# mj129/Tramba

Measured on AMD Instinct MI355X. Metric: images/sec fwd Tramba-V 384x384, higher is better.
Workload: dtype bf16; 1 GPU; Tramba-V (VMamba-B encoder) 384x384 bf16 inference, batch 4 per GPU, random-init weights (seed 1026), randn images; global_batch=4, launch=hipGraph replay, decoder guide branches on a side stream

## Files before the change

include/tramba_hip.h:

```cpp
#ifndef TRAMBA_HIP_H
#define TRAMBA_HIP_H

#include <stddef.h>
#include <stdint.h>

#ifdef __cplusplus
extern "C" {
#endif

typedef enum { TRAMBA_F32 = 0, TRAMBA_F16 = 1, TRAMBA_BF16 = 2 } tramba_dtype;

typedef enum {
    TRAMBA_SCAN_RASTER = 0,
    TRAMBA_SCAN_LINE = 1,
    TRAMBA_SCAN_HELIX = 2,
    TRAMBA_SCAN_WINDOW = 3,
    TRAMBA_SCAN_DILATION = 4
} tramba_scan_family;

typedef enum { TRAMBA_ACT_NONE = 0, TRAMBA_ACT_SILU = 1, TRAMBA_ACT_GELU = 2,
               TRAMBA_ACT_SIGMOID_GATE = 3 ,
               TRAMBA_ACT_GELU_GRAD_MUL = 4
             } tramba_act;

#define TRAMBA_OK 0
#define TRAMBA_ERR_ARG (-1)
#define TRAMBA_ERR_UNSUPPORTED (-2)
#define TRAMBA_ERR_HIP (-3)

const char *tramba_last_error(void);
int tramba_abi_version(void);
int tramba_device_error(void);
int tramba_profile_enable(int which, int enable);
int tramba_profile_read(int which, double *total_ms, double *total_bytes);
int tramba_profile_min_units(int which, double min_units);
int tramba_tune_set(int knob, int value);
int tramba_tune_get(int knob);
#define TRAMBA_TUNE_MERGE_FORM 0
#define TRAMBA_TUNE_SCAN_FORM 1
#define TRAMBA_TUNE_SCAN_W 2
#define TRAMBA_TUNE_GEMM_TILE 3
#define TRAMBA_TUNE_MAILBOX_SKIP 4
#define TRAMBA_TUNE_DW_FORM 6
#define TRAMBA_TUNE_DW_ROWS 7
#define TRAMBA_TUNE_COUNT 8
#define TRAMBA_PROF_SCAN_BOUNDARY 0
#define TRAMBA_PROF_SCAN_FUSED 1
#define TRAMBA_PROF_GEMM 2
#define TRAMBA_PROF_MERGE 3
#define TRAMBA_PROF_SCAN_BWD 4
#define TRAMBA_PROF_WGRAD 5
#define TRAMBA_PROF_LAYERNORM 6
#define TRAMBA_PROF_DW 7
#define TRAMBA_PROF_COUNT 8

int tramba_scan_family_k(int family);
int tramba_default_window(int h);
int tramba_scan_table(int family, int h, int w, int param, int32_t *out);
int tramba_scan_table_inverse(const int32_t *table, int k, int l, int32_t *inv_ptr, int32_t *inv_idx);

int tramba_selective_scan_nchunk(int l, int io_dtype);
int tramba_selective_scan_fwd(const void *u, const void *delta, const float *A, const void *Bm,
                              const void *Cm, const float *D, const float *delta_bias, void *out,
                              float *ckpt, int batch, int kd, int k, int n, int l, int io_dtype,
                              int out_dtype, int delta_softplus, void *stream);
int tramba_selective_scan_bwd(const void *u, const void *delta, const float *A, const void *Bm,
                              const void *Cm, const float *D, const float *delta_bias,
                              const float *dout, const float *ckpt, void *du, void *ddelta,
                              float *dA, float *dB, float *dC, float *dD, float *ddelta_bias,
                              int batch, int kd, int k, int n, int l, int io_dtype,
                              int delta_softplus, int ncopy, void *stream);

int tramba_cross_scan(const void *x, const int32_t *table, void *xs, int batch, int c, int l, int k,
                      int dtype, void *stream);
int tramba_cross_merge(const void *ys, const int32_t *inv_ptr, const int32_t *inv_idx, void *y,
                       int batch, int c, int l, int k, int dtype, void *stream);

int tramba_ss2d_group_stride(int r);
size_t tramba_ss2d_scan_workspace(int batch, int l, int d, int k);
int tramba_ss2d_scan_cl(const void *x, const float *xdbl, const int32_t *table, const float *dt_w,
                        const float *dt_bias, const float *A, const float *Ds, void *ys, void *workspace,
                        size_t workspace_bytes, int batch, int l, int d, int k, int r, int dtype,
                        int ys_dtype, float *states, int a_log, void *stream);
size_t tramba_ss2d_scan_bwd_workspace(int batch, int l, int d, int k);
int tramba_ss2d_scan_bwd_cl(const void *x, const float *xdbl, const int32_t *table, const float *dt_w,
                            const float *dt_bias, const float *A, const float *Ds, const void *gym, void *gu,
                            void *graw, float *gB, float *gC, int bc_stride, float *gpar, void *workspace,
                            size_t workspace_bytes, int have_states, int batch, int l, int d, int k, int r, int dtype,
                            int gym_dtype, int flags, void *stream);
#define TRAMBA_SCAN_BWD_A_LOG 1
#define TRAMBA_SCAN_BWD_BC_PARTIALS 2
int tramba_ss2d_bwd_prep_cl(const float *xdbl, const int32_t *table, const float *bpart, const float *cpart, void *ranks,
                            float *gseq, int batch, int l, int k, int r, int ctiles, int dtype, void *stream);
int tramba_ss2d_bwd_assemble_cl(const float *gseq, const int32_t *inv_ptr, const int32_t *inv_idx, void *out, int batch,
                                int l, int k, int r, int dtype, void *stream);
int tramba_ss2d_merge_norm_cl(const void *ys, const int32_t *inv_ptr, const int32_t *inv_idx,
                              const float *ln_w, const float *ln_b, void *y, int batch, int l, int d,
                              int k, float eps, int act, int ys_dtype, int dtype, void *stream);
// ... 152 lines not shown
```

tramba_amd/csrc/linear.hip:

```cpp
#include <stdlib.h>
#include <string.h>

#include <type_traits>

#include "common.h"

namespace tramba {

typedef __attribute__((ext_vector_type(8))) short frag8_t;
typedef __attribute__((ext_vector_type(8))) _Float16 frag8h_t;
typedef __attribute__((ext_vector_type(16))) float acc16_t;

template <typename T> struct Mfma;
template <> struct Mfma<__hip_bfloat16> {
    static constexpr int KSTEP = 16;
    using frag = frag8_t;
    static __device__ __forceinline__ acc16_t run(frag a, frag b, acc16_t c)
    {
        typedef __attribute__((ext_vector_type(8))) __bf16 bf8;
        return __builtin_amdgcn_mfma_f32_32x32x16_bf16(__builtin_bit_cast(bf8, a), __builtin_bit_cast(bf8, b), c, 0, 0, 0);
    }
};
template <> struct Mfma<__half> {
    static constexpr int KSTEP = 16;
// ... 715 lines not shown
        acc[0][0] = Mfma<T>::run(b[2], a[2], acc[0][0]);
        asm volatile("s_waitcnt lgkmcnt(0)" : "+v"(a[3]), "+v"(b[3]) : : "memory");
        acc[0][0] = Mfma<T>::run(b[3], a[3], acc[0][0]);
    };
    int kt0 = 0;
    for (; kt0 + NSTG <= nk; kt0 += NSTG) {
        kstep(kt0, std::integral_constant<int, 0>{});
        kstep(kt0 + 1, std::integral_constant<int, 1>{});
        if constexpr (NSTG > 2) kstep(kt0 + 2, std::integral_constant<int, 2>{});
        if constexpr (NSTG > 3) kstep(kt0 + 3, std::integral_constant<int, 3>{});
        if constexpr (NSTG > 4) {
            kstep(kt0 + 4, std::integral_constant<int, 4>{});
            kstep(kt0 + 5, std::integral_constant<int, 5>{});
            kstep(kt0 + 6, std::integral_constant<int, 6>{});
            kstep(kt0 + 7, std::integral_constant<int, 7>{});
        }
    }
    if (kt0 < nk) kstep(kt0, std::integral_constant<int, 0>{});
    if constexpr (NSTG > 2) {
        if (kt0 + 1 < nk) kstep(kt0 + 1, std::integral_constant<int, 1>{});
    }
    if constexpr (NSTG > 3) {
        if (kt0 + 2 < nk) kstep(kt0 + 2, std::integral_constant<int, 2>{});
    }
    if constexpr (NSTG > 4) {
        if (kt0 + 3 < nk) kstep(kt0 + 3, std::integral_constant<int, 3>{});
        if (kt0 + 4 < nk) kstep(kt0 + 4, std::integral_constant<int, 4>{});
        if (kt0 + 5 < nk) kstep(kt0 + 5, std::integral_constant<int, 5>{});
        if (kt0 + 6 < nk) kstep(kt0 + 6, std::integral_constant<int, 6>{});
    }
    __syncthreads();
    if constexpr (LNIN) {
        float2 *rowstat = reinterpret_cast<float2 *>(lds + LDS_BYTES);
#pragma unroll
        for (int i = 0; i < 2; ++i) {
            float s1 = rs1[i], s2 = rs2[i];
#pragma unroll
            for (int m = 1; m < 8; m <<= 1) {
                s1 += __shfl_xor(s1, m, 64);
                s2 += __shfl_xor(s2, m, 64);
            }
            const float mean = s1 / (float)K;
            const float var = fmaxf(s2 / (float)K - mean * mean, 0.f);
            if ((tid & 7) == 0) rowstat[(tid >> 3) + 32 * i] = make_float2(mean, rsqrtf(var + li.eps));
        }
        tile_epilogue<T, TO, BM, BN>(acc, lds, bias, res, y, M, N, act, m0, n0, li.colsum,
                                     reinterpret_cast<const float2 *>(lds + LDS_BYTES));
    } else {
        tile_epilogue<T, TO, BM, BN>(acc, lds, bias, res, y, M, N, act, m0, n0, nullptr, nullptr, DUAL ? y_pre : nullptr);
    }
#endif
}

#define TRAMBA_DSR128_(OUT, ADDR, OFF) asm volatile("ds_read_b128 %0, %1 offset:" #OFF : "=v"(OUT) : "v"(ADDR) : "memory")
template <typename T, typename TO, int NSTG, bool LNIN = false, bool DUAL = false>
__global__ __launch_bounds__(512) void linear_pc_kernel(const T *__restrict__ x, const T *__restrict__ w,
                                                       const float *__restrict__ bias, const T *__restrict__ res,
                                                       TO *__restrict__ y, long M, int N, int K, int act,
                                                       LnIn li = LnIn{nullptr, 0.f}, TO *__restrict__ y_pre = nullptr)
{
#if defined(__HIP_DEVICE_COMPILE__)
    constexpr int BM = 64, BN = 64;
    constexpr int TILE_BYTES = (BM + BN) * kBK * 2;
    constexpr int EPI_BYTES = BM * (BN + 4) * 4;
    constexpr int LDS_BYTES = NSTG * TILE_BYTES > EPI_BYTES ? NSTG * TILE_BYTES : EPI_BYTES;
    static_assert(NSTG == 3 || NSTG == 4, "stage index = kt % NSTG with the loop unrolled by NSTG");
    __shared__ __attribute__((aligned(1024))) unsigned char lds[LDS_BYTES + (LNIN ? BM * 8 : 0)];
    typedef __attribute__((address_space(3))) void lds_void;

    const int tid = threadIdx.x, lane = tid & 63;
    const int wave = __builtin_amdgcn_readfirstlane(tid >> 6);
    const bool loader = wave >= 4;
    const int cw = wave & 3;
    const int wm = cw >> 1, wn = cw & 1;
    const int r32 = lane & 31, hi = lane >> 5;
    long m0;
    int n0;
    {
        const unsigned nblk = gridDim.x * gridDim.y, lin = blockIdx.y * gridDim.x + blockIdx.x;
        const unsigned q = nblk >> 3, r = nblk & 7, xcd = lin & 7, slot = lin >> 3;
        const unsigned t = xcd * q + (xcd < r ? xcd : r) + slot;
        m0 = (long)(t / gridDim.x) * BM;
        n0 = (int)(t % gridDim.x) * BN;
    }
    const int nk = K / kBK;
    const unsigned rowb = (unsigned)K * 2u;
    const long mrows = M - m0 < BM ? M - m0 : BM;
    const int nrows = N - n0 < BN ? N - n0 : BN;
    const bool stage_b = cw >= 2;
    const __amdgpu_buffer_rsrc_t rs = stage_b ? make_rsrc(w + (long)n0 * K, (unsigned)nrows * rowb)
                                              : make_rsrc(x + m0 * K, (unsigned)mrows * rowb);
    unsigned voff[4];
#pragma unroll
    for (int j = 0; j < 4; ++j) {
        const int row = ((cw & 1) * 4 + j) * 8 + (lane >> 3);
        const int c = (lane & 7) ^ ((row >> 1) & 7);
        voff[j] = (unsigned)row * rowb + (unsigned)c * 16u;
    }
    unsigned char *mine = lds + (stage_b ? BM * kBK * 2 : 0) + (cw & 1) * 4096;
    auto issue = [&](int kt, int stg) {
        const unsigned so = (unsigned)kt * (kBK * 2);
#pragma unroll
        for (int j = 0; j < 4; ++j)
            __builtin_amdgcn_raw_ptr_buffer_load_lds(rs, (lds_void *)(mine + stg * TILE_BYTES + j * 1024), 16, voff[j], so, 0,
                                                     0);
    };
    const unsigned lbase = (unsigned)(size_t)(__attribute__((address_space(3))) unsigned char *)lds;
    unsigned aad[4], bad[4];
    {
        const int ra_ = wm * 32 + r32, rb_ = wn * 32 + r32;
        const unsigned a0 = lbase + (unsigned)(ra_ * 128 + ((hi ^ ((ra_ >> 1) & 7)) * 16));
        const unsigned b0 = lbase + (unsigned)(BM * kBK * 2 + rb_ * 128 + ((hi ^ ((rb_ >> 1) & 7)) * 16));
#pragma unroll
        for (int kk = 0; kk < 4; ++kk) {
            aad[kk] = a0 ^ (unsigned)(kk * 32);
            bad[kk] = b0 ^ (unsigned)(kk * 32);
        }
    }
    acc16_t acc[1][1];
#pragma unroll
    for (int r = 0; r < 16; ++r) acc[0][0][r] = 0.f;
    const int lt = tid & 255;
    float rs1[2] = {0.f, 0.f}, rs2[2] = {0.f, 0.f};
    const unsigned sad = lbase + (unsigned)((lt >> 3) * 128 + (lt & 7) * 16);

    constexpr int DEPTH = NSTG - 1;
    if (loader) {
#pragma unroll
        for (int t = 0; t < DEPTH; ++t)
            if (t < nk) issue(t, t);
    }
    auto kstep = [&](int kt, auto stg_c) {
        constexpr int STG = decltype(stg_c)::value;
        if (loader) {
            const int later = nk - 1 - kt;
            if (later >= DEPTH - 1) {
                if constexpr (DEPTH == 2) asm volatile("s_waitcnt vmcnt(4)" ::: "memory");
                else asm volatile("s_waitcnt vmcnt(8)" ::: "memory");
            } else {
                switch (later) {
                case 0: asm volatile("s_waitcnt vmcnt(0)" ::: "memory"); break;
                default: asm volatile("s_waitcnt vmcnt(4)" ::: "memory"); break;
                }
            }
        }
        __builtin_amdgcn_s_barrier();
        asm volatile("" ::: "memory");
        if (loader) {
            if (kt + DEPTH < nk) issue(kt + DEPTH, (STG + DEPTH) % NSTG);
        } else {
            frag8_t a[4], b[4];
            v4u_t sv[2];
            if constexpr (LNIN) {
                if constexpr (STG == 0) { TRAMBA_DSR128_(sv[0], sad, 0); TRAMBA_DSR128_(sv[1], sad, 4096); }
                else if constexpr (STG == 1) { TRAMBA_DSR128_(sv[0], sad, 16384); TRAMBA_DSR128_(sv[1], sad, 20480); }
                else if constexpr (STG == 2) { TRAMBA_DSR128_(sv[0], sad, 32768); TRAMBA_DSR128_(sv[1], sad, 36864); }
                else { TRAMBA_DSR128_(sv[0], sad, 49152); TRAMBA_DSR128_(sv[1], sad, 53248); }
            }
#define TRAMBA_RD_STG_(S)                                                                            \
    TRAMBA_DSR128_(a[0], aad[0], S); TRAMBA_DSR128_(b[0], bad[0], S); TRAMBA_DSR128_(a[1], aad[1], S); \
    TRAMBA_DSR128_(b[1], bad[1], S); TRAMBA_DSR128_(a[2], aad[2], S); TRAMBA_DSR128_(b[2], bad[2], S); \
    TRAMBA_DSR128_(a[3], aad[3], S); TRAMBA_DSR128_(b[3], bad[3], S)
// ... 366 lines not shown
    return ncw;
}

template <typename T, int K, bool LNIN, bool DUAL, bool RES>
static void launch_ws(int ncw, const void *x, const void *w, const float *bias, const void *res, void *y, long m, int n, int act,
                      LnIn li, void *y_pre, hipStream_t s)
{
    const int npanel = n / (128 * ncw);
    const long t32 = (m + 31) / 32;
    const long resident = 256L * (K == 128 ? 3 : 2);
    long gt = resident / npanel;
    if (gt > t32) gt = t32;
    if (gt < 1) gt = 1;
    dim3 grid((unsigned)(gt * npanel)), block(256);
#define WS_(NCW_)                                                                                                      \
    hipLaunchKernelGGL((linear_ws_kernel<T, K, NCW_, LNIN, DUAL, RES>), grid, block, 0, s, (const T *)x, (const T *)w, bias, \
                       (const T *)res, (T *)y, m, n, act, li, (T *)y_pre, npanel, (int)gt)
    if constexpr (K == 128) {
        if (ncw == 2) { WS_(2); } else { WS_(1); }
    } else {
        WS_(1);
    }
#undef WS_
}

template <typename T, bool LNIN, bool DUAL>
static void launch_ws_k(int ncw, const void *x, const void *w, const float *bias, const void *res, void *y, long m, int n, int k,
                        int act, LnIn li, void *y_pre, hipStream_t s)
{
    if (k == 128) {
        if (res) { if constexpr (!DUAL) launch_ws<T, 128, LNIN, false, true>(ncw, x, w, bias, res, y, m, n, act, li, y_pre, s); }
        else launch_ws<T, 128, LNIN, DUAL, false>(ncw, x, w, bias, res, y, m, n, act, li, y_pre, s);
    } else {
        if (res) { if constexpr (!DUAL) launch_ws<T, 256, LNIN, false, true>(ncw, x, w, bias, res, y, m, n, act, li, y_pre, s); }
        else launch_ws<T, 256, LNIN, DUAL, false>(ncw, x, w, bias, res, y, m, n, act, li, y_pre, s);
    }
}

constexpr int DMA_SHORT_K = 256;

enum GemmKind { GEMM_PLAIN = 0, GEMM_LN = 1, GEMM_DUAL = 2, GEMM_TWO_SRC, GEMM_CONV };
enum class GemmForm {
    WS,
    PC3, PC4,
    DMA2, DMA3, DMA4,
    LEAN,
    TILED128, TILED64, TILED64_PF3
};
struct GemmPlan {
    GemmForm form;
    int ncw;
};

static GemmPlan gemm_plan(GemmKind kind, long m, int n, int k, int act, bool same_dtype)
{
    if (kind == GEMM_TWO_SRC) return {GemmForm::LEAN, 0};
    if (kind == GEMM_CONV || k % 64 != 0 || (double)k * 2.0 * 128.0 >= 2147483648.0) {
        const long big = ((m + 127) / 128) * ((n + 127) / 128);
        if (big >= 2048 && k >= 1024) return {GemmForm::TILED128, 0};
        return {k <= 128 ? GemmForm::TILED64 : GemmForm::TILED64_PF3, 0};
    }
    int tune = tramba_tune_get(TRAMBA_TUNE_GEMM_TILE);
    if (tune == 7 && kind != GEMM_PLAIN) tune = 0;
    if (tune == 0 || tune == 19) {
        const bool ws_act = act == TRAMBA_ACT_NONE || act == TRAMBA_ACT_GELU || act == TRAMBA_ACT_SILU;
        const int ncw = same_dtype && ws_act ? ws_ncw(m, n, k) : 0;
        if (ncw && (tune == 19 ? m >= 64 : ws_rule(m, n, k, kind))) return {GemmForm::WS, ncw};
    }
    switch (tune) {
    case 7: return {GemmForm::DMA4, 0};
    case 13: return {GemmForm::DMA2, 0};
    case 14: return {GemmForm::DMA3, 0};
    case 16: return {GemmForm::PC3, 0};
    case 17: return {GemmForm::PC4, 0};
    }
    const long tiles64 = ((m + 63) / 64) * ((n + 63) / 64);
    const int pc = tune == 18 ? 0 : pc_rule(tiles64, k, kind);
    if (pc) return {pc == 4 ? GemmForm::PC4 : GemmForm::PC3, 0};
    if (k <= DMA_SHORT_K && tiles64 >= 1024) return {GemmForm::DMA2, 0};
    if (kind == GEMM_PLAIN && tiles64 <= 256 && k >= 1024) return {GemmForm::DMA4, 0};
    return {GemmForm::DMA3, 0};
}

struct GemmArgs {
    const void *x, *w;
    const float *bias;
    const void *res;
    void *y;
    long m;
    int n, k, act;
    LnIn li{nullptr, 0.f};
    void *y_pre = nullptr;
    const void *x2 = nullptr;
    int k1 = 0;
    ConvGeom cg{0, 0, 0, 0, 0};
};

template <typename T, typename TO, bool LNIN = false, bool DUAL = false, bool CONV = false>
static void launch_gemm(const GemmPlan &p, const GemmArgs &a, hipStream_t s)
{
    const T *x = (const T *)a.x, *w = (const T *)a.w, *res = (const T *)a.res;
    TO *y = (TO *)a.y, *y_pre = (TO *)a.y_pre;
    const long m = a.m;
    const int n = a.n, k = a.k, act = a.act;
    const dim3 g64((n + 63) / 64, (unsigned)((m + 63) / 64)), g128((n + 127) / 128, (unsigned)((m + 127) / 128));
    switch (p.form) {
    case GemmForm::WS:
        launch_ws_k<T, LNIN, DUAL>(p.ncw, a.x, a.w, a.bias, a.res, a.y, m, n, k, act, a.li, a.y_pre, s);
        break;
    case GemmForm::PC3:
        hipLaunchKernelGGL((linear_pc_kernel<T, TO, 3, LNIN, DUAL>), g64, dim3(512), 0, s, x, w, a.bias, res, y, m, n, k, act, a.li, y_pre);
        break;
    case GemmForm::PC4:
        hipLaunchKernelGGL((linear_pc_kernel<T, TO, 4, LNIN, DUAL>), g64, dim3(512), 0, s, x, w, a.bias, res, y, m, n, k, act, a.li, y_pre);
        break;
    case GemmForm::DMA2:
        hipLaunchKernelGGL((linear_dma_kernel<T, TO, 2, LNIN, DUAL>), g64, dim3(256), 0, s, x, w, a.bias, res, y, m, n, k, act, a.li, y_pre);
        break;
    case GemmForm::DMA3:
        hipLaunchKernelGGL((linear_dma_kernel<T, TO, 3, LNIN, DUAL>), g64, dim3(256), 0, s, x, w, a.bias, res, y, m, n, k, act, a.li, y_pre);
        break;
    case GemmForm::DMA4:
        if constexpr (!LNIN && !DUAL)
            hipLaunchKernelGGL((linear_dma_kernel<T, TO, 4>), g64, dim3(256), 0, s, x, w, a.bias, res, y, m, n, k, act, a.li, y_pre);
        break;
    case GemmForm::LEAN:
        hipLaunchKernelGGL((linear_lean_kernel<T, TO, 64, 64, 1>), g64, dim3(256), 0, s, x, w, a.bias, res, y, m, n, k, act,
                           (const T *)a.x2, a.k1);
        break;
    case GemmForm::TILED128:
        hipLaunchKernelGGL((linear_tiled_kernel<T, TO, 128, 128, 2, CONV>), g128, dim3(256), 0, s, x, w, a.bias, res, y, m, n, k, act, a.cg);
        break;
    case GemmForm::TILED64:
        hipLaunchKernelGGL((linear_tiled_kernel<T, TO, 64, 64, 1, CONV>), g64, dim3(256), 0, s, x, w, a.bias, res, y, m, n, k, act, a.cg);
        break;
    case GemmForm::TILED64_PF3:
        hipLaunchKernelGGL((linear_tiled_kernel<T, TO, 64, 64, 3, CONV>), g64, dim3(256), 0, s, x, w, a.bias, res, y, m, n, k, act, a.cg);
        break;
    }
}

template <bool LNIN = false>
static void launch_gemm16(const GemmPlan &p, const GemmArgs &a, int dtype, int out_dtype, hipStream_t s)
{
    if (dtype == TRAMBA_BF16) {
        if (out_dtype == TRAMBA_F32) launch_gemm<__hip_bfloat16, float, LNIN>(p, a, s);
        else launch_gemm<__hip_bfloat16, __hip_bfloat16, LNIN>(p, a, s);
    } else {
        if (out_dtype == TRAMBA_F32) launch_gemm<__half, float, LNIN>(p, a, s);
        else launch_gemm<__half, __half, LNIN>(p, a, s);
    }
}

template <typename TO>
__global__ __launch_bounds__(256) void linear32_kernel(const float *__restrict__ x, const float *__restrict__ w,
                                                      const float *__restrict__ bias, const float *__restrict__ res,
                                                      TO *__restrict__ y, long M, int N, int K, int act)
{
    const int lane = threadIdx.x & 63, wave = threadIdx.x >> 6;
    const long m0 = (long)blockIdx.y * 128 + (wave >> 1) * 64;
    const int n0 = blockIdx.x * 128 + (wave & 1) * 64;
    if (m0 >= M || n0 >= N) return;
    acc16_t acc[2][2];
#pragma unroll
    for (int i = 0; i < 2; ++i)
#pragma unroll
        for (int j = 0; j < 2; ++j)
#pragma unroll
// ... 114 lines not shown
                 "linear2_cl: tensors must be 16-byte aligned");
    TRAMBA_CHECK((m + 63) / 64 <= 65535 && (double)k * 2.0 * 128.0 < 2147483648.0, "linear2_cl: shape exceeds this build's limits");
    hipStream_t s = (hipStream_t)stream;
    ProfScope prof(TRAMBA_PROF_GEMM, s, 2.0 * (double)m * n * k);
    GemmArgs a{x1, w, bias, residual, y, m, n, k, act};
    a.x2 = x2;
    a.k1 = k1;
    launch_gemm16(gemm_plan(GEMM_TWO_SRC, m, n, k, act, out_dtype == dtype), a, dtype, out_dtype, s);
    TRAMBA_LAUNCH_CHECK();
    return TRAMBA_OK;
}

extern "C" int tramba_expand_norm_head_cl(const void *x, const void *w, const float *ln_w, const float *ln_b,
                                          const float *head_w, float head_b, float *y, int batch, int h, int wd, int cin,
                                          int p, float eps, int dtype, void *stream)
{
    TRAMBA_CHECK(x && w && ln_w && ln_b && head_w && y, "expand_norm_head_cl: null tensor");
    TRAMBA_CHECK(batch > 0 && h > 0 && wd > 0 && cin > 0 && p > 0, "expand_norm_head_cl: empty shape");
    TRAMBA_CHECK(dtype == TRAMBA_BF16 || dtype == TRAMBA_F16, "expand_norm_head_cl: 16-bit dtypes only");
    TRAMBA_CHECK(cin % 64 == 0, "expand_norm_head_cl: Cin=%d must be a multiple of 64", cin);
    TRAMBA_CHECK(aligned16(x) && aligned16(w), "expand_norm_head_cl: tensors must be 16-byte aligned");
    const long m = (long)batch * h * wd;
    const int n = p * p * 128;
    TRAMBA_CHECK(m < 2147483647L && (m + 63) / 64 <= 65535, "expand_norm_head_cl: too many pixels");
    hipStream_t s = (hipStream_t)stream;
    ProfScope prof(TRAMBA_PROF_GEMM, s, 2.0 * (double)m * n * cin);
    const LnHead hd{ln_w, ln_b, head_w, head_b, eps, h, wd, p, y};
    dim3 grid((unsigned)(n / 128), (unsigned)((m + 63) / 64)), block(256);
    if (dtype == TRAMBA_BF16) {
        using T = __hip_bfloat16;
        hipLaunchKernelGGL((linear_lean_kernel<T, T, 64, 128, 1, true>), grid, block, 0, s, (const T *)x, (const T *)w,
                           (const float *)nullptr, (const T *)nullptr, (T *)nullptr, m, n, cin, 0, (const T *)nullptr, 0, hd);
    } else {
        using T = __half;
        hipLaunchKernelGGL((linear_lean_kernel<T, T, 64, 128, 1, true>), grid, block, 0, s, (const T *)x, (const T *)w,
                           (const float *)nullptr, (const T *)nullptr, (T *)nullptr, m, n, cin, 0, (const T *)nullptr, 0, hd);
    }
    TRAMBA_LAUNCH_CHECK();
    return TRAMBA_OK;
}

extern "C" int tramba_conv3x3s2_cl(const void *x, const void *w, const float *bias, void *y, int batch, int hin,
                                   int win, int cin, int cout, int dtype, void *stream)
{
    TRAMBA_CHECK(x && w && y, "conv3x3s2_cl: null tensor");
    TRAMBA_CHECK(batch > 0 && hin > 0 && win > 0 && cin > 0 && cout > 0, "conv3x3s2_cl: empty shape");
    TRAMBA_CHECK(cin % 64 == 0, "conv3x3s2_cl: Cin=%d must be a multiple of 64", cin);
    TRAMBA_CHECK(dtype == TRAMBA_BF16 || dtype == TRAMBA_F16, "conv3x3s2_cl: bf16/f16 only (fp32 convs run on MIOpen)");
    TRAMBA_CHECK(aligned16(x) && aligned16(w) && aligned16(y), "conv3x3s2_cl: tensors must be 16-byte aligned");
    ConvGeom cg{hin, win, cin, (hin + 1) / 2, (win + 1) / 2};
    const long m = (long)batch * cg.hout * cg.wout;
    TRAMBA_CHECK((m + 63) / 64 <= 65535, "conv3x3s2_cl: too many output pixels");
    hipStream_t s = (hipStream_t)stream;
    const GemmPlan p = gemm_plan(GEMM_CONV, m, cout, 9 * cin, TRAMBA_ACT_NONE, true);
    GemmArgs a{x, w, bias, nullptr, y, m, cout, 9 * cin, TRAMBA_ACT_NONE};
    a.cg = cg;
    if (dtype == TRAMBA_BF16) launch_gemm<__hip_bfloat16, __hip_bfloat16, false, false, true>(p, a, s);
    else launch_gemm<__half, __half, false, false, true>(p, a, s);
    TRAMBA_LAUNCH_CHECK();
    return TRAMBA_OK;
}

extern "C" int tramba_linear_dual_cl(const void *x, const void *w, const float *bias, void *y_pre, void *y_act, int64_t m,
                                     int n, int k, int act, int dtype, void *stream)
{
    TRAMBA_CHECK(x && w && y_pre && y_act, "linear_dual_cl: null tensor");
    TRAMBA_CHECK(m > 0 && n > 0 && k > 0, "linear_dual_cl: empty shape");
    TRAMBA_CHECK(dtype == TRAMBA_BF16 || dtype == TRAMBA_F16, "linear_dual_cl: 16-bit activations only");
    TRAMBA_CHECK(act == TRAMBA_ACT_GELU || act == TRAMBA_ACT_SILU, "linear_dual_cl: act must be GELU or SiLU");
    TRAMBA_CHECK(k % 64 == 0 && n % 8 == 0 && (double)k * 2.0 * 128.0 < 2147483648.0 && (m + 63) / 64 <= 65535,
                 "linear_dual_cl: needs K %% 64 == 0, N %% 8 == 0");
    TRAMBA_CHECK(aligned16(x) && aligned16(w) && aligned16(y_pre) && aligned16(y_act), "linear_dual_cl: 16-byte alignment");
    hipStream_t s = (hipStream_t)stream;
    ProfScope prof(TRAMBA_PROF_GEMM, s, 2.0 * (double)m * n * k);
    const GemmPlan p = gemm_plan(GEMM_DUAL, m, n, k, act, true);
    GemmArgs a{x, w, bias, nullptr, y_act, m, n, k, act};
    a.y_pre = y_pre;
    if (dtype == TRAMBA_BF16) launch_gemm<__hip_bfloat16, __hip_bfloat16, false, true>(p, a, s);
    else launch_gemm<__half, __half, false, true>(p, a, s);
    TRAMBA_LAUNCH_CHECK();
    return TRAMBA_OK;
}
```

tramba_amd/csrc/ss2d_fused.hip:

```cpp
#include <stdlib.h>
#include <string.h>

#include <type_traits>

#include "common.h"
#include "norm.h"

namespace tramba {

constexpr int kMaxW = 8;

typedef __attribute__((ext_vector_type(8))) short frag8_t;
typedef __attribute__((ext_vector_type(8))) __bf16 bf16x8_t;
typedef __attribute__((ext_vector_type(16))) float acc16_t;

constexpr int kTP = 32;

__host__ __device__ inline int xdbl_rank_pad(int r) { return (r + 7) & ~7; }
__host__ __device__ inline int xdbl_group_stride(int r) { return xdbl_rank_pad(r) + 4; }
inline double rg_bytes(int r) { return 4.0 * xdbl_group_stride(r); }

template <bool SPLIT>
__device__ __forceinline__ void pack_frag(const float (&v)[8], frag8_t &hi, frag8_t &lo)
{
// ... 1628 lines not shown
    case 1: BWD_(T, 1, SP_); break;    \
    case 2: BWD_(T, 2, SP_); break;    \
    case 3: BWD_(T, 3, SP_); break;    \
    default: BWD_(T, 4, SP_); break;   \
    }
    if (dtype == TRAMBA_F32) { BWD_NK_(float, true) }
    else if (dtype == TRAMBA_BF16) { BWD_NK_(__hip_bfloat16, false) }
    else if (dtype == TRAMBA_F16) { BWD_NK_(__half, false) }
    else {
        set_error("ss2d_scan_bwd_cl: bad dtype %d", dtype);
        return TRAMBA_ERR_ARG;
    }
#undef BWD_NK_
#undef BWD_
#undef BWD_G_
    TRAMBA_LAUNCH_CHECK();
    return TRAMBA_OK;
}

extern "C" int tramba_ss2d_merge_norm_cl(const void *ys, const int32_t *inv_ptr, const int32_t *inv_idx,
                                         const float *ln_w, const float *ln_b, void *y, int batch, int l,
                                         int d, int k, float eps, int act, int ys_dtype, int dtype,
                                         void *stream)
{
    return tramba_ss2d_merge_grad_cl(ys, inv_ptr, inv_idx, ln_w, ln_b, y, nullptr, nullptr, batch, l, d, k, eps, act, ys_dtype,
                                     dtype, stream);
}

extern "C" int tramba_ss2d_merge_grad_cl(const void *ys, const int32_t *inv_ptr, const int32_t *inv_idx,
                                         const float *ln_w, const float *ln_b, void *y, const void *addend,
                                         const void *zpre, int batch, int l, int d, int k, float eps, int act,
                                         int ys_dtype, int dtype, void *stream)
{
    TRAMBA_CHECK(ys && inv_ptr && inv_idx && y && (eps < 0.f || (ln_w && ln_b)), "ss2d_merge_norm_cl: null tensor");
    TRAMBA_CHECK((!addend && !zpre) || (eps < 0.f && zpre && aligned16(zpre) && (!addend || aligned16(addend))),
                 "ss2d_merge_grad_cl: the SiLU-gradient epilogue belongs to a merge-only call (eps < 0) and needs zpre");
    TRAMBA_CHECK(batch > 0 && l > 0 && d > 0 && k > 0, "ss2d_merge_norm_cl: empty shape");
    TRAMBA_CHECK(ys_dtype == TRAMBA_F32 || ys_dtype == dtype, "ss2d_merge_norm_cl: ys must be f32 or dtype");
    hipStream_t s = (hipStream_t)stream;
    const long npix = (long)batch * l;
    TRAMBA_CHECK(npix < 2147483647L, "ss2d_merge_norm_cl: B*L exceeds the 32-bit pixel index of this build");
    int v = (d % 4 == 0) ? 4 : ((d % 2 == 0) ? 2 : 1);
    TRAMBA_CHECK((d + kWave * v - 1) / (kWave * v) <= kNormMaxIt, "ss2d_merge_norm_cl: D=%d too large", d);
    TRAMBA_CHECK(aligned16(ys) && aligned16(y), "ss2d_merge_norm_cl: tensors must be 16-byte aligned");
    const int nit_need = (d + kWave * v - 1) / (kWave * v);
    const int nit = nit_need <= 1 ? 1 : (nit_need <= 2 ? 2 : (nit_need <= 4 ? 4 : 8));
    ProfScope prof(TRAMBA_PROF_MERGE, s, (double)batch * k * l * (double)d * dtype_size(ys_dtype) +
                                              (double)batch * l * (double)d * dtype_size(dtype));
    const bool sum_only = eps < 0.f;
    const int tune = tramba_tune_get(TRAMBA_TUNE_MERGE_FORM);
    const bool stream_ok = !sum_only && nit <= 2 && k <= 8 && (double)k * l * d * 4.0 < 4294967296.0;
    const bool stream_form = stream_ok && (tune == 2 || (tune == 0 && k <= 4 && npix >= 8192));
    const bool wide = k > 4;
    const int pw = wide ? 4 : 16;
    const int nchunk = (l + pw - 1) / pw;
    const long nwaves = (long)batch * nchunk;
    int hs = 0;
    if (wide) {
        hs = 1;
        while ((long)hs * hs < l) ++hs;
        if ((long)hs * hs != l || hs % pw != 0) hs = 0;
    }
    const bool split_form = !sum_only && !stream_form && tune != 1 && (ys_dtype == TRAMBA_F32 || k <= 4) && nit >= 4 &&
                            npix <= 16384;
    if (!stream_form && !split_form) {
        const int vd = norm_vec(d, ys_dtype == TRAMBA_F32 ? 4 : 8);
        const int nd_need = (d + kWave * vd - 1) / (kWave * vd);
        TRAMBA_CHECK(nd_need <= kNormMaxIt, "ss2d_merge_norm_cl: D=%d too large", d);
        TRAMBA_CHECK((double)k * l * d * 4.0 < 4294967296.0, "ss2d_merge_norm_cl: K*L*D too large for 32-bit offsets");
        const int nd = nd_need <= 1 ? 1 : (nd_need <= 2 ? 2 : (nd_need <= 4 ? 4 : 8));
        int hh = 1;
        while ((long)hh * hh < l) ++hh;
        if ((long)hh * hh != l) hh = 0;
        dim3 gridd((unsigned)((npix + 3) / 4)), blockd(256);
#define DEEP_(TY, T, V_, N_)                                                                                      \
    hipLaunchKernelGGL((ss2d_merge_norm_deep_kernel<TY, T, V_, N_>), gridd, blockd, 0, s, (const TY *)ys, inv_ptr, \
                       inv_idx, ln_w, ln_b, (T *)y, npix, batch, l, d, k, hh, eps, act, (const T *)addend, (const T *)zpre)
#define DEEP_N_(TY, T, V_)                    \
    if (nd == 1) { DEEP_(TY, T, V_, 1); }     \
    else if (nd == 2) { DEEP_(TY, T, V_, 2); } \
    else if (nd == 4) { DEEP_(TY, T, V_, 4); } \
    else { DEEP_(TY, T, V_, 8); }
#define DEEP_V_(TY, T)                                                  \
    if (vd == 8) {                                                      \
        if constexpr (sizeof(TY) == 2) { DEEP_N_(TY, T, 8) }            \
    } else if (vd == 4) { DEEP_N_(TY, T, 4) }                           \
    else if (vd == 2) { DEEP_N_(TY, T, 2) }                             \
    else { DEEP_N_(TY, T, 1) }
        TRAMBA_DISPATCH_DTYPE(dtype, T, {
            if (ys_dtype == TRAMBA_F32) { DEEP_V_(float, T) } else { DEEP_V_(T, T) }
        });
#undef DEEP_V_
#undef DEEP_N_
#undef DEEP_
        TRAMBA_LAUNCH_CHECK();
        return TRAMBA_OK;
    }
    dim3 grid(stream_form ? (unsigned)((nwaves + 3) / 4) : (unsigned)npix), block(256);
#define GO_(TY, T, V_, N_)                                                                                    \
    if (split_form)                                                                                           \
        hipLaunchKernelGGL((ss2d_merge_norm_split_kernel<TY, T, V_, (N_ >= 4 ? N_ : 4), 4>), grid, block, 0, s, \
                           (const TY *)ys, inv_ptr, inv_idx, ln_w, ln_b, (T *)y, npix, l, d, k, eps, act);    \
    else if (wide)                                                                                            \
        hipLaunchKernelGGL((ss2d_merge_norm_stream_kernel<TY, T, V_, (N_ <= 2 ? N_ : 2), 8>), grid, block, 0, s, \
                           (const TY *)ys, inv_ptr, inv_idx, ln_w, ln_b, (T *)y, nwaves, nchunk, pw, l, d, k, eps, \
                           act, batch, hs);                                                                   \
    else                                                                                                      \
// ... 24 lines not shown
```

tramba_amd/hip.py:

```python
import ctypes
import os
import threading
import weakref

import numpy as np
import torch

_HERE = os.path.dirname(os.path.abspath(__file__))
LIB_PATH = os.path.join(_HERE, "_lib", "libtramba_hip.so")

F32, F16, BF16 = 0, 1, 2
ACT_NONE, ACT_SILU, ACT_GELU, ACT_SIGMOID_GATE, ACT_GELU_GRAD_MUL = 0, 1, 2, 3, 4
SCAN_RASTER, SCAN_LINE, SCAN_HELIX, SCAN_WINDOW, SCAN_DILATION = range(5)
FAMILY = {"raster": SCAN_RASTER, "line": SCAN_LINE, "helix": SCAN_HELIX, "window": SCAN_WINDOW,
          "dilation": SCAN_DILATION}
PROF_SCAN_BOUNDARY, PROF_SCAN_FUSED, PROF_GEMM, PROF_MERGE, PROF_SCAN_BWD, PROF_WGRAD, PROF_LAYERNORM, PROF_DW = 0, 1, 2, 3, 4, 5, 6, 7

_DT = {torch.float32: F32, torch.float16: F16, torch.bfloat16: BF16}

c_int, c_i64, c_f, c_vp = ctypes.c_int, ctypes.c_int64, ctypes.c_float, ctypes.c_void_p

SIGNATURES = {
    "tramba_last_error": (ctypes.c_char_p, []),
    "tramba_abi_version": (c_int, []),
# ... 172 lines not shown
        return conv
    _f32_cache[key] = (ver, conv, ref)
    return conv


_table_cache = {}


def default_window(h: int) -> int:
    return lib().tramba_default_window(h)


def scan_table_host(family: str, h: int, w: int = None, param: int = 0) -> np.ndarray:
    w = h if w is None else w
    fam = FAMILY[family]
    k = _check(lib().tramba_scan_family_k(fam), "scan_family_k")
    out = np.empty((k, h * w), dtype=np.int32)
    _check(lib().tramba_scan_table(fam, h, w, param, out.ctypes.data), f"scan_table({family},{h})")
    return out


def scan_table_inverse_host(table: np.ndarray):
    k, l = table.shape
    table = np.ascontiguousarray(table, dtype=np.int32)
    ptr = np.empty(l + 1, dtype=np.int32)
    idx = np.empty(k * l, dtype=np.int32)
    _check(lib().tramba_scan_table_inverse(table.ctypes.data, k, l, ptr.ctypes.data, idx.ctypes.data),
           "scan_table_inverse")
    return ptr, idx


class ScanOrder:

    def __init__(self, family, h, w, param, device):
        host = scan_table_host(family, h, w, param)
        ptr, idx = scan_table_inverse_host(host)
        self.family, self.h, self.w, self.k, self.l = family, h, w, host.shape[0], host.shape[1]
        self.table = torch.from_numpy(host).to(device)
        self.inv_ptr = torch.from_numpy(ptr).to(device)
        self.inv_idx = torch.from_numpy(idx).to(device)
        if not torch.cuda.is_current_stream_capturing():
            torch.cuda.current_stream(device).synchronize()


def scan_order(family: str, h: int, w: int, device, param: int = 0) -> ScanOrder:
    key = (family, h, w, param, str(device))
    so = _table_cache.get(key)
    if so is None:
        so = _table_cache[key] = ScanOrder(family, h, w, param, device)
    return so


TUNE_MERGE_FORM, TUNE_SCAN_FORM, TUNE_SCAN_W, TUNE_GEMM_TILE, TUNE_MAILBOX_SKIP, TUNE_DW_FORM, TUNE_DW_ROWS = 0, 1, 2, 3, 4, 6, 7


def device_error():
    _check(lib().tramba_device_error(), "device_error")


def tune_set(knob: int, value: int):
    _check(lib().tramba_tune_set(knob, value), "tune_set")


def profile_enable(which: int, on: bool):
    _check(lib().tramba_profile_enable(which, int(on)), "profile_enable")


def profile_min_units(which: int, min_units: float):
    _check(lib().tramba_profile_min_units(which, float(min_units)), "profile_min_units")


def profile_read(which: int):
    ms, units = ctypes.c_double(), ctypes.c_double()
    n = _check(lib().tramba_profile_read(which, ctypes.byref(ms), ctypes.byref(units)), "profile_read")
    return n, ms.value, units.value


def selective_scan_nchunk(l: int, dtype: torch.dtype) -> int:
    return lib().tramba_selective_scan_nchunk(l, _DT[dtype])


def selective_scan_fwd(u, delta, A, B, C, D, delta_bias, delta_softplus=True, oflex=True, want_ckpt=True):
    _dev(u, delta, A, B, C, D, delta_bias)
    nb, kd, l = u.shape
    k, n = B.shape[1], B.shape[2]
    if delta.shape != u.shape or A.shape != (kd, n) or B.shape != (nb, k, n, l) or C.shape != B.shape:
        raise TrambaHipError(f"selective_scan_fwd: inconsistent shapes u{tuple(u.shape)} delta{tuple(delta.shape)} "
                             f"A{tuple(A.shape)} B{tuple(B.shape)} C{tuple(C.shape)}")
    if not (delta.dtype == B.dtype == C.dtype == u.dtype):
        raise TrambaHipError("selective_scan_fwd: u, delta, B, C must share a dtype")
    out = torch.empty((nb, kd, l), dtype=torch.float32 if oflex else u.dtype, device=u.device)
    ckpt = None
    if want_ckpt:
        ckpt = torch.empty((nb, kd, selective_scan_nchunk(l, u.dtype), n), dtype=torch.float32, device=u.device)
    A, D, delta_bias = _f32(A), _f32(D), _f32(delta_bias)
    _check(lib().tramba_selective_scan_fwd(
        _ptr(u), _ptr(delta), _ptr(A), _ptr(B), _ptr(C), _ptr(D), _ptr(delta_bias), _ptr(out), _ptr(ckpt),
        nb, kd, k, n, l, dt(u), dt(out), int(delta_softplus), _stream()), "selective_scan_fwd")
    return out, ckpt


def selective_scan_bwd(u, delta, A, B, C, D, delta_bias, dout, ckpt, delta_softplus=True):
    _dev(u, delta, A, B, C, D, delta_bias, dout, ckpt)
    nb, kd, l = u.shape
    k, n = B.shape[1], B.shape[2]
    A32, D32, b32 = _f32(A), _f32(D), _f32(delta_bias)
# ... 1098 lines not shown
```

Baseline: 864.2 img/s.

## Route two-source and conv3x3 GEMMs through producer-consumer DMA kernel; adapt merge chunk width

Extends the producer-consumer buffer-to-LDS GEMM kernel with two A-source modes. One is a two-tensor concatenated K, which avoids materialising a concat. The other is an implicit 3x3 stride-2 conv that computes per-row halo coordinates and masks out-of-bounds loads via the buffer offset high bit. gemm_plan now sends GEMM_TWO_SRC and GEMM_CONV to PC3/PC4 instead of the LEAN/TILED64 kernels. Separately, the merge-norm chunk width now halves until there are enough waves, with a new tune knob to override it. This adds template variants and relies on out-of-range buffer loads returning zero for padding.

```diff
diff --git a/include/tramba_hip.h b/include/tramba_hip.h
--- a/include/tramba_hip.h
+++ b/include/tramba_hip.h
@@ -43,7 +43,8 @@
 #define TRAMBA_TUNE_MAILBOX_SKIP 4
 #define TRAMBA_TUNE_DW_FORM 6
 #define TRAMBA_TUNE_DW_ROWS 7
-#define TRAMBA_TUNE_COUNT 8
+#define TRAMBA_TUNE_MERGE_PW 8
+#define TRAMBA_TUNE_COUNT 9
 #define TRAMBA_PROF_SCAN_BOUNDARY 0
 #define TRAMBA_PROF_SCAN_FUSED 1
 #define TRAMBA_PROF_GEMM 2
diff --git a/tramba_amd/csrc/linear.hip b/tramba_amd/csrc/linear.hip
--- a/tramba_amd/csrc/linear.hip
+++ b/tramba_amd/csrc/linear.hip
@@ -791,12 +791,21 @@
 #endif
 }
 
+enum { A_PLAIN = 0, A_TWO = 1, A_CONV = 2 };
+struct ASrc {
+    const void *x2;
+    int k1;
+    ConvGeom cg;
+    unsigned abytes;
+};
+
 #define TRAMBA_DSR128_(OUT, ADDR, OFF) asm volatile("ds_read_b128 %0, %1 offset:" #OFF : "=v"(OUT) : "v"(ADDR) : "memory")
-template <typename T, typename TO, int NSTG, bool LNIN = false, bool DUAL = false>
-__global__ __launch_bounds__(512) void linear_pc_kernel(const T *__restrict__ x, const T *__restrict__ w,
+template <typename T, typename TO, int NSTG, bool LNIN = false, bool DUAL = false, int ASRC = A_PLAIN>
+__global__ __launch_bounds__(512, ASRC == A_CONV && NSTG == 3 ? 6 : 1) void linear_pc_kernel(const T *__restrict__ x, const T *__restrict__ w,
                                                        const float *__restrict__ bias, const T *__restrict__ res,
                                                        TO *__restrict__ y, long M, int N, int K, int act,
-                                                       LnIn li = LnIn{nullptr, 0.f}, TO *__restrict__ y_pre = nullptr)
+                                                       LnIn li = LnIn{nullptr, 0.f}, TO *__restrict__ y_pre = nullptr,
+                                                       ASrc as = ASrc{nullptr, 0, ConvGeom{0, 0, 0, 0, 0}, 0u})
 {
 #if defined(__HIP_DEVICE_COMPILE__)
     constexpr int BM = 64, BN = 64;
@@ -827,26 +836,97 @@
     const long mrows = M - m0 < BM ? M - m0 : BM;
     const int nrows = N - n0 < BN ? N - n0 : BN;
     const bool stage_b = cw >= 2;
-    const __amdgpu_buffer_rsrc_t rs = stage_b ? make_rsrc(w + (long)n0 * K, (unsigned)nrows * rowb)
-                                              : make_rsrc(x + m0 * K, (unsigned)mrows * rowb);
+    __amdgpu_buffer_rsrc_t rs, rsx;
     unsigned voff[4];
-#pragma unroll
-    for (int j = 0; j < 4; ++j) {
-        const int row = ((cw & 1) * 4 + j) * 8 + (lane >> 3);
-        const int c = (lane & 7) ^ ((row >> 1) & 7);
-        voff[j] = (unsigned)row * rowb + (unsigned)c * 16u;
+    unsigned lx[4] = {0u, 0u, 0u, 0u}, ly[4] = {0u, 0u, 0u, 0u};
+    unsigned(&voff2)[4] = lx;
+    unsigned(&chy)[4] = lx, (&cwx)[4] = ly;
+    int nsw = nk;
+    unsigned hlim = 0xffffffffu, wlim = 0xffffffffu;
+    int ccs = 0, cdy = 0, cdx = 0;
+    if constexpr (ASRC == A_TWO) {
+        const int ka = as.k1;
+        const unsigned rowa = (unsigned)ka * 2u, rowa2 = (unsigned)(K - ka) * 2u;
+        rs = stage_b ? make_rsrc(w + (long)n0 * K, (unsigned)nrows * rowb) : make_rsrc(x + m0 * ka, (unsigned)mrows * rowa);
+        rsx = stage_b ? rs : make_rsrc((const T *)as.x2 + m0 * (K - ka), (unsigned)mrows * rowa2);
+        if (!stage_b) nsw = ka / kBK;
+#pragma unroll
+        for (int j = 0; j < 4; ++j) {
+            const int row = ((cw & 1) * 4 + j) * 8 + (lane >> 3);
+            const int c = (lane & 7) ^ ((row >> 1) & 7);
+            voff[j] = (unsigned)row * (stage_b ? rowb : rowa) + (unsigned)c * 16u;
+            voff2[j] = (unsigned)row * (stage_b ? rowb : rowa2) + (unsigned)c * 16u;
+        }
+    } else if constexpr (ASRC == A_CONV) {
+        rs = stage_b ? make_rsrc(w + (long)n0 * K, (unsigned)nrows * rowb) : make_rsrc(x, as.abytes);
+        if (!stage_b) {
+            hlim = (unsigned)as.cg.hin;
+            wlim = (unsigned)as.cg.win;
+        }
+#pragma unroll
+        for (int j = 0; j < 4; ++j) {
+            const int row = ((cw & 1) * 4 + j) * 8 + (lane >> 3);
+            const int c = (lane & 7) ^ ((row >> 1) & 7);
+            if (stage_b) {
+                voff[j] = (unsigned)row * rowb + (unsigned)c * 16u;
+                chy[j] = cwx[j] = 0u;
+            } else {
+                const long gr = m0 + row;
+                const bool ok = gr < M;
+                const unsigned pix = ok ? (unsigned)gr : 0u;
+                const unsigned wo = pix % (unsigned)as.cg.wout, t = pix / (unsigned)as.cg.wout;
+                const unsigned ho = t % (unsigned)as.cg.hout, b = t / (unsigned)as.cg.hout;
+                chy[j] = (unsigned)(ok ? 2 * (int)ho - 1 : -4);
+                cwx[j] = (unsigned)(2 * (int)wo - 1);
+                voff[j] = ((b * (unsigned)as.cg.hin + chy[j]) * (unsigned)as.cg.win + cwx[j]) * ((unsigned)as.cg.cin * 2u) +
+                          (unsigned)c * 16u;
+            }
+        }
+    } else {
+        rs = stage_b ? make_rsrc(w + (long)n0 * K, (unsigned)nrows * rowb) : make_rsrc(x + m0 * K, (unsigned)mrows * rowb);
+#pragma unroll
+        for (int j = 0; j < 4; ++j) {
+            const int row = ((cw & 1) * 4 + j) * 8 + (lane >> 3);
+            const int c = (lane & 7) ^ ((row >> 1) & 7);
+            voff[j] = (unsigned)row * rowb + (unsigned)c * 16u;
+        }
     }
     unsigned char *mine = lds + (stage_b ? BM * kBK * 2 : 0) + (cw & 1) * 4096;
     auto issue = [&](int kt, int stg) {
-        const unsigned so = (unsigned)kt * (kBK * 2);
-#pragma unroll
-        for (int j = 0; j < 4; ++j)
-            __builtin_amdgcn_raw_ptr_buffer_load_lds(rs, (lds_void *)(mine + stg * TILE_BYTES + j * 1024), 16, voff[j], so, 0,
-                                                     0);
+        if constexpr (ASRC == A_TWO) {
+            const bool first = kt < nsw;
+            const __amdgpu_buffer_rsrc_t rsel = first ? rs : rsx;
+            const unsigned so = (unsigned)(first ? kt : kt - nsw) * (kBK * 2);
+#pragma unroll
+            for (int j = 0; j < 4; ++j)
+                __builtin_amdgcn_raw_ptr_buffer_load_lds(rsel, (lds_void *)(mine + stg * TILE_BYTES + j * 1024), 16,
+                                                         first ? voff[j] : voff2[j], so, 0, 0);
+        } else if constexpr (ASRC == A_CONV) {
+            const unsigned so = stage_b ? (unsigned)kt * (kBK * 2)
+                                        : (unsigned)((cdy * as.cg.win + cdx) * as.cg.cin + ccs * kBK) * 2u;
+#pragma unroll
+            for (int j = 0; j < 4; ++j) {
+                const unsigned hy = chy[j] + (unsigned)cdy, wx = cwx[j] + (unsigned)cdx;
+                unsigned out = (hy < hlim && wx < wlim) ? 0u : 1u;
+                asm volatile("" : "+v"(out));
+                __builtin_amdgcn_raw_ptr_buffer_load_lds(rs, (lds_void *)(mine + stg * TILE_BYTES + j * 1024), 16,
+                                                         (voff[j] + so) | (out << 31), 0, 0, 0);
+            }
+            if (++ccs == as.cg.cin / kBK) {
+                ccs = 0;
+                if (++cdx == 3) { cdx = 0; ++cdy; }
+            }
+        } else {
+            const unsigned so = (unsigned)kt * (kBK * 2);
+#pragma unroll
+            for (int j = 0; j < 4; ++j)
+                __builtin_amdgcn_raw_ptr_buffer_load_lds(rs, (lds_void *)(mine + stg * TILE_BYTES + j * 1024), 16, voff[j], so,
+                                                         0, 0);
+        }
     };
     const unsigned lbase = (unsigned)(size_t)(__attribute__((address_space(3))) unsigned char *)lds;
-    unsigned aad[4], bad[4];
-    {
+    unsigned(&aad)[4] = lx, (&bad)[4] = ly;
+    if (ASRC == A_PLAIN || !loader) {
         const int ra_ = wm * 32 + r32, rb_ = wn * 32 + r32;
         const unsigned a0 = lbase + (unsigned)(ra_ * 128 + ((hi ^ ((ra_ >> 1) & 7)) * 16));
         const unsigned b0 = lbase + (unsigned)(BM * kBK * 2 + rb_ * 128 + ((hi ^ ((rb_ >> 1) & 7)) * 16));
@@ -1319,15 +1399,20 @@
     int ncw;
 };
 
-static GemmPlan gemm_plan(GemmKind kind, long m, int n, int k, int act, bool same_dtype)
-{
+static GemmPlan gemm_plan(GemmKind kind, long m, int n, int k, int act, bool same_dtype, bool a_dma = true)
+{
+    int tune = tramba_tune_get(TRAMBA_TUNE_GEMM_TILE);
+    if ((kind == GEMM_TWO_SRC || kind == GEMM_CONV) && a_dma && tune != 18 && k % 64 == 0 &&
+        (double)k * 2.0 * 128.0 < 2147483648.0) {
+        const long tiles64 = ((m + 63) / 64) * ((n + 63) / 64);
+        return {pc_rule(tiles64, k, GEMM_PLAIN) == 4 ? GemmForm::PC4 : GemmForm::PC3, 0};
+    }
     if (kind == GEMM_TWO_SRC) return {GemmForm::LEAN, 0};
     if (kind == GEMM_CONV || k % 64 != 0 || (double)k * 2.0 * 128.0 >= 2147483648.0) {
         const long big = ((m + 127) / 128) * ((n + 127) / 128);
         if (big >= 2048 && k >= 1024) return {GemmForm::TILED128, 0};
         return {k <= 128 ? GemmForm::TILED64 : GemmForm::TILED64_PF3, 0};
     }
-    int tune = tramba_tune_get(TRAMBA_TUNE_GEMM_TILE);
     if (tune == 7 && kind != GEMM_PLAIN) tune = 0;
     if (tune == 0 || tune == 19) {
         const bool ws_act = act == TRAMBA_ACT_NONE || act == TRAMBA_ACT_GELU || act == TRAMBA_ACT_SILU;
@@ -1361,6 +1446,7 @@
     const void *x2 = nullptr;
     int k1 = 0;
     ConvGeom cg{0, 0, 0, 0, 0};
+    unsigned abytes = 0;
 };
 
 template <typename T, typename TO, bool LNIN = false, bool DUAL = false, bool CONV = false>
@@ -1376,11 +1462,26 @@
         launch_ws_k<T, LNIN, DUAL>(p.ncw, a.x, a.w, a.bias, a.res, a.y, m, n, k, act, a.li, a.y_pre, s);
         break;
     case GemmForm::PC3:
-        hipLaunchKernelGGL((linear_pc_kernel<T, TO, 3, LNIN, DUAL>), g64, dim3(512), 0, s, x, w, a.bias, res, y, m, n, k, act, a.li, y_pre);
+    case GemmForm::PC4: {
+        const bool four = p.form == GemmForm::PC4;
+        if constexpr (CONV) {
+            const ASrc as{nullptr, 0, a.cg, a.abytes};
+            if (four) hipLaunchKernelGGL((linear_pc_kernel<T, TO, 4, false, false, A_CONV>), g64, dim3(512), 0, s, x, w, a.bias, res, y, m, n, k, act, a.li, y_pre, as);
+            else hipLaunchKernelGGL((linear_pc_kernel<T, TO, 3, false, false, A_CONV>), g64, dim3(512), 0, s, x, w, a.bias, res, y, m, n, k, act, a.li, y_pre, as);
+            break;
+        }
+        if constexpr (!LNIN && !DUAL) {
+            if (a.x2) {
+                const ASrc as{a.x2, a.k1, a.cg, 0u};
+                if (four) hipLaunchKernelGGL((linear_pc_kernel<T, TO, 4, false, false, A_TWO>), g64, dim3(512), 0, s, x, w, a.bias, res, y, m, n, k, act, a.li, y_pre, as);
+                else hipLaunchKernelGGL((linear_pc_kernel<T, TO, 3, false, false, A_TWO>), g64, dim3(512), 0, s, x, w, a.bias, res, y, m, n, k, act, a.li, y_pre, as);
+                break;
+            }
+        }
+        if (four) hipLaunchKernelGGL((linear_pc_kernel<T, TO, 4, LNIN, DUAL>), g64, dim3(512), 0, s, x, w, a.bias, res, y, m, n, k, act, a.li, y_pre);
+        else hipLaunchKernelGGL((linear_pc_kernel<T, TO, 3, LNIN, DUAL>), g64, dim3(512), 0, s, x, w, a.bias, res, y, m, n, k, act, a.li, y_pre);
         break;
-    case GemmForm::PC4:
-        hipLaunchKernelGGL((linear_pc_kernel<T, TO, 4, LNIN, DUAL>), g64, dim3(512), 0, s, x, w, a.bias, res, y, m, n, k, act, a.li, y_pre);
-        break;
+    }
     case GemmForm::DMA2:
         hipLaunchKernelGGL((linear_dma_kernel<T, TO, 2, LNIN, DUAL>), g64, dim3(256), 0, s, x, w, a.bias, res, y, m, n, k, act, a.li, y_pre);
         break;
@@ -1601,9 +1702,11 @@
     const long m = (long)batch * cg.hout * cg.wout;
     TRAMBA_CHECK((m + 63) / 64 <= 65535, "conv3x3s2_cl: too many output pixels");
     hipStream_t s = (hipStream_t)stream;
-    const GemmPlan p = gemm_plan(GEMM_CONV, m, cout, 9 * cin, TRAMBA_ACT_NONE, true);
+    const double xbytes = (double)batch * hin * win * cin * 2.0;
+    const GemmPlan p = gemm_plan(GEMM_CONV, m, cout, 9 * cin, TRAMBA_ACT_NONE, true, xbytes < 2147483648.0);
     GemmArgs a{x, w, bias, nullptr, y, m, cout, 9 * cin, TRAMBA_ACT_NONE};
     a.cg = cg;
+    a.abytes = (unsigned)xbytes;
     if (dtype == TRAMBA_BF16) launch_gemm<__hip_bfloat16, __hip_bfloat16, false, false, true>(p, a, s);
     else launch_gemm<__half, __half, false, false, true>(p, a, s);
     TRAMBA_LAUNCH_CHECK();
diff --git a/tramba_amd/csrc/ss2d_fused.hip b/tramba_amd/csrc/ss2d_fused.hip
--- a/tramba_amd/csrc/ss2d_fused.hip
+++ b/tramba_amd/csrc/ss2d_fused.hip
@@ -1704,7 +1704,12 @@
     const bool stream_ok = !sum_only && nit <= 2 && k <= 8 && (double)k * l * d * 4.0 < 4294967296.0;
     const bool stream_form = stream_ok && (tune == 2 || (tune == 0 && k <= 4 && npix >= 8192));
     const bool wide = k > 4;
-    const int pw = wide ? 4 : 16;
+    const int pw_tune = tramba_tune_get(TRAMBA_TUNE_MERGE_PW);
+    TRAMBA_CHECK(pw_tune == 0 || pw_tune == 4 || pw_tune == 8 || pw_tune == 16, "TRAMBA_TUNE_MERGE_PW %d: 0, 4, 8 or 16", pw_tune);
+    int pw = wide ? 4 : 16;
+    if (pw_tune > 0) pw = pw_tune;
+    else
+        while (pw > 4 && (long)batch * ((l + pw - 1) / pw) < 4096) pw >>= 1;
     const int nchunk = (l + pw - 1) / pw;
     const long nwaves = (long)batch * nchunk;
     int hs = 0;
diff --git a/tramba_amd/hip.py b/tramba_amd/hip.py
--- a/tramba_amd/hip.py
+++ b/tramba_amd/hip.py
@@ -248,6 +248,7 @@
 
 
 TUNE_MERGE_FORM, TUNE_SCAN_FORM, TUNE_SCAN_W, TUNE_GEMM_TILE, TUNE_MAILBOX_SKIP, TUNE_DW_FORM, TUNE_DW_ROWS = 0, 1, 2, 3, 4, 6, 7
+TUNE_MERGE_PW = 8
 
 
 def device_error():
```

Measured after the change: 877.4 img/s, median of 6. +1.5%, better.
